# Gabrielcb/DaliID

Measured on AMD Instinct MI355X. Metric: images/sec (train step), higher is better.
Workload: dtype bf16; 1 GPU; configs[1]: ResNet-50 ReID bf16 256x128, PK batch 16x16=256 per GPU, center+proxy heads, Adam, EMA; global_batch=256, per_gpu_batch=256, parallelism=dp1

## Files before the change

daliid_amd/csrc/conv.hip:

```cpp
#include "gemm_tile.h"
#include "kernels.h"
#include <cstdlib>
#include <type_traits>
#include <vector>
#include <string>
#include <cstdio>

namespace dali {

__device__ __forceinline__ void decode_pixel(const GatherGeom& g, int p, int& n, int& ho, int& wo) {
    if (g.lhw >= 0 && g.lw >= 0) {
        n = p >> g.lhw;
        const int rem = p & ((1 << g.lhw) - 1);
        ho = rem >> g.lw;
        wo = rem & ((1 << g.lw) - 1);
    } else {
        const int hw = g.Hout * g.Wout;
        n = p / hw;
        const int rem = p - n * hw;
        ho = rem / g.Wout;
        wo = rem - ho * g.Wout;
    }
}

// ... 2294 lines not shown
    GRID_XCD,
    GRID_CLASSES,
    GRID_CUS,
    GRID_HALO,
    GRID_SPLITS,
    GRID_SPLITS8,
};
struct GemmKernel {
    const void* fn;
    int block;
    int lds;
    int tm, tn;
    GemmGrid grid;
    int plan_wgs = 0;
    int f1_rb = 0;
    mutable DeviceOnce once{};
};
template <class F> static const void* kfn(F* f) { return reinterpret_cast<const void*>(f); }
constexpr int ring_lds(int tm, int tn, int k_tile, int stages) { return (tm + tn) * k_tile * 2 * stages; }
constexpr int REG128_LDS = GemmCfg<128, 128, 1, 1, 1>::LDS_BYTES, REG64_LDS = GemmCfg<64, 256, 1, 1, 1>::LDS_BYTES;
constexpr int DMA128_LDS = REG128_LDS / 2 * 3, DMA64_LDS = REG64_LDS / 2 * 3;
constexpr int HALO64_LDS = (3 * 64 * 64 + HALO64_PX * 64) * 2;

static const GemmKernel
    CONV128_BN{kfn(&igemm_conv_kernel<128, 128, true>), 256, REG128_LDS, 128, 128, GRID_XCD},
    CONV128{kfn(&igemm_conv_kernel<128, 128, false>), 256, REG128_LDS, 128, 128, GRID_XCD},
    DMA128{kfn(&igemm_conv_dma_kernel<128, 128, 3>), 256, DMA128_LDS, 128, 128, GRID_XCD},
    DMA128_LIN{kfn(&igemm_conv_dma_kernel<128, 128, 3, 1>), 256, DMA128_LDS, 128, 128, GRID_XCD},
    DMA128_FUSED{kfn(&igemm_conv_dma_kernel<128, 128, 3, 3>), 256, DMA128_LDS, 128, 128, GRID_XCD},
    DMA128_CLS{kfn(&igemm_conv_dma_kernel<128, 128, 3, 4>), 256, DMA128_LDS, 128, 128, GRID_CLASSES},
// ... 11 lines not shown
    WG128_FUSED{kfn(&igemm_conv_wg_kernel<2, 4, 3, 3>), 512, ring_lds(128, 256, 32, 3), 128, 256, GRID_XCD},
    WG128_CLS{kfn(&igemm_conv_wg_kernel<2, 4, 3, 4>), 512, ring_lds(128, 256, 32, 3), 128, 256, GRID_CLASSES},
    WG256{kfn(&igemm_conv_wg_kernel<4, 4, 4>), 1024, ring_lds(256, 256, 32, 4), 256, 256, GRID_XCD},
    K64S{kfn(&igemm_conv_k64s_kernel<2, 4, 8, 3>), 1024, ring_lds(128, 256, 64, 3), 128, 256, GRID_XCD},
    K64S_LIN{kfn(&igemm_conv_k64s_kernel<2, 4, 8, 3, 4, 4, 1>), 1024, ring_lds(128, 256, 64, 3), 128, 256, GRID_XCD},
    K64S_LEAN{kfn(&igemm_conv_k64s_kernel<2, 4, 8, 3, 4, 4, 5>), 1024, ring_lds(128, 256, 64, 3), 128, 256, GRID_XCD},
    K64S_SRC2{kfn(&igemm_conv_k64s_kernel<2, 4, 8, 3, 4, 4, 0, true>), 1024, ring_lds(128, 256, 64, 3), 128, 256, GRID_XCD},
    K64{kfn(&igemm_conv_k64_kernel<4, 4, 2>), 1024, ring_lds(256, 256, 64, 2), 256, 256, GRID_XCD},
    K64_LIN{kfn(&igemm_conv_k64_kernel<4, 4, 2, 4, 4, 1>), 1024, ring_lds(256, 256, 64, 2), 256, 256, GRID_XCD},
    K64_FUSED{kfn(&igemm_conv_k64_kernel<4, 4, 2, 4, 4, 3>), 1024, ring_lds(256, 256, 64, 2), 256, 256, GRID_XCD},
    K64_CLS{kfn(&igemm_conv_k64_kernel<4, 4, 2, 4, 4, 4>), 1024, ring_lds(256, 256, 64, 2), 256, 256, GRID_CLASSES},
    K64_SRC2{kfn(&igemm_conv_k64_kernel<4, 4, 2, 4, 4, 0, true>), 1024, ring_lds(256, 256, 64, 2), 256, 256, GRID_XCD},
    K64_FUSED_SRC2{kfn(&igemm_conv_k64_kernel<4, 4, 2, 4, 4, 3, true>), 1024, ring_lds(256, 256, 64, 2), 256, 256, GRID_XCD},
    K64_320{kfn(&igemm_conv_k64_kernel<4, 4, 2, 4, 5, 1>), 1024, ring_lds(256, 320, 64, 2), 256, 320, GRID_XCD};

template <int RB, bool RES, bool OM, bool BITS, bool SRC2 = false>
static GemmKernel f1_kernel() {
    return {kfn(&fused1x1_persist_kernel<3, RB, RES, OM, BITS, SRC2>), (F1_NC + F1_NP + F1_NR) * 64, f1_lds_bytes(3, RB, RB == 2 ? 128 : F1_KMAX),
            F1_TM, F1_TN, GRID_CUS, 0, RB};
}
static const GemmKernel F1[2][2][2][2] = {
    {{{f1_kernel<2, false, false, false, true>(), f1_kernel<2, false, false, true>()}, {f1_kernel<2, false, true, false>(), f1_kernel<2, false, true, true>()}},
     {{f1_kernel<2, true, false, false>(), f1_kernel<2, true, false, true>()}, {f1_kernel<2, true, true, false>(), f1_kernel<2, true, true, true>()}}},
    {{{f1_kernel<1, false, false, false, true>(), f1_kernel<1, false, false, true>()}, {f1_kernel<1, false, true, false>(), f1_kernel<1, false, true, true>()}},
     {{f1_kernel<1, true, false, false>(), f1_kernel<1, true, false, true>()}, {f1_kernel<1, true, true, false>(), f1_kernel<1, true, true, true>()}}}};

static const GemmKernel
    WG_BN{kfn(&igemm_wgrad_kernel<true>), 256, 0, 128, 128, GRID_SPLITS},
    WG_PLAIN{kfn(&igemm_wgrad_kernel<false>), 256, 0, 128, 128, GRID_SPLITS},
    WG_3X3{kfn(&igemm_wgrad3x3_kernel<3>), 512, 3 * W3_STAGE * 2, 128, 9 * 64, GRID_SPLITS8, 256};
static const GemmKernel WG_DMA[2] = {
    {kfn(&igemm_wgrad_dma_kernel<false>), 256, 0, 128, 128, GRID_SPLITS8},
    {kfn(&igemm_wgrad_dma_kernel<true>), 256, 0, 128, 128, GRID_SPLITS8}};
static const GemmKernel WG_WG[2] = {
    {kfn(&igemm_wgrad_wg_kernel<2, 4, 3>), 512, ring_lds(128, 256, 32, 3), 128, 256, GRID_SPLITS8, 512},
    {kfn(&igemm_wgrad_wg_kernel<2, 4, 3, true>), 512, ring_lds(128, 256, 32, 3), 128, 256, GRID_SPLITS8, 512}};
static const GemmKernel WG_P[2][2] = {
    {{kfn(&igemm_wgrad_p_kernel<2, 4, 4, 4, 8, 6>), 1024, ring_lds(128, 256, 32, 6), 128, 256, GRID_SPLITS8, 256},
     {kfn(&igemm_wgrad_p_kernel<2, 4, 4, 4, 8, 6, true>), 1024, ring_lds(128, 256, 32, 6), 128, 256, GRID_SPLITS8, 256}},
    {{kfn(&igemm_wgrad_p_kernel<1, 4, 8, 4, 4, 6>), 512, ring_lds(128, 256, 32, 6), 128, 256, GRID_SPLITS8, 256},
// ... 2 lines not shown
struct GemmChoice {
    const GemmKernel* k = nullptr;
    int tiles_m = 0, tiles_n = 0, lds = 0, class_grid = 0;
    unsigned grid = 0;
    int rc = DALI_OK, why_arg = 0;
    const char* why = nullptr;
    GemmChoice() = default;
    GemmChoice(int rc_, const char* why_, int why_arg_ = 0) : rc(rc_), why_arg(why_arg_), why(why_) {}
    int refuse() const { set_error(why, why_arg); return rc; }
};
static GemmChoice gemm_place(const GemmKernel& k, int rows, int cols, int mult, int Ck) {
    GemmChoice c;
    c.k = &k;
    c.tiles_m = (rows + k.tm - 1) / k.tm;
    c.tiles_n = (cols + k.tn - 1) / k.tn;
    c.lds = k.f1_rb ? f1_lds_bytes(3, k.f1_rb, Ck) : k.lds;
    switch (k.grid) {
        case GRID_XCD: c.grid = xcd_tile_grid(c.tiles_m, c.tiles_n); break;
        case GRID_CLASSES: c.class_grid = xcd_tile_grid(c.tiles_m, c.tiles_n); c.grid = mult * c.class_grid; break;
        case GRID_CUS: c.grid = mult; break;
        case GRID_HALO: c.grid = c.tiles_n; break;
        case GRID_SPLITS: c.grid = c.tiles_m * c.tiles_n * mult; break;
        case GRID_SPLITS8: c.grid = (c.tiles_m * c.tiles_n * mult + 7) / 8 * 8; break;
    }
    return c;
}
template <class Args>
static int gemm_launch(hipStream_t st, const GemmChoice& c, Args& args) {
    const GemmKernel& k = *c.k;
    DeviceOnce::Guard once(k.once);
    if (k.lds > 64 * 1024 && once.first()) {
// ... 31 lines not shown
    if (!n_cus) {
        int dev = 0, v = 0;
        if (hipGetDevice(&dev) != hipSuccess || hipDeviceGetAttribute(&v, hipDeviceAttributeMultiprocessorCount, dev) != hipSuccess) { set_error("conv: device query failed"); return -1; }
        n_cus = v > 8 ? v & ~7 : 8;
    }
    return n_cus;
}
static bool f1_fills(int Cm, int P, int n_cus) {
    const int tiles_m = Cm / F1_TM, tiles_n = (P + F1_TN - 1) / F1_TN;
    return n_cus > 0 && (long long)tiles_m * tiles_n >= 2ll * n_cus && (n_cus / 8) % tiles_m == 0;
}
static bool cat_act_ok(int Cm, int c1, int c2, int P, int parts, int n_cus) {
    const int K = parts * (c1 + c2);
    if (parts != 1 && parts != 2) return false;
    if ((c1 & 63) || (c2 & 63) || (Cm % 128) || !dma_addressable((long long)P * Cm * 2) || !dma_addressable((long long)P * K * 2)) return false;
    if (K <= F1_KMAX) return f1_fills(Cm, P, n_cus);
    return parts == 1 && K >= 1024 && conv_pick_cfg(Cm, P, K) == CONV_256x256;
}
bool conv_cat_act_supported(int Cm, int c1, int c2, int P, int parts) { return cat_act_ok(Cm, c1, c2, P, parts, f1_cu_count()); }

static GemmChoice conv_choose(const IGemmArgs& a, int n_cus) {
    const GatherGeom& g = a.g;
    const bool in_bn = a.in_scale != nullptr, narrow = a.Cm <= 64, dma_ok = conv_dma_ok(a);
    const int K = g.nr * g.ns * g.Ck;
    const bool fused = a.out_scale || a.out_shift || a.out_relu || a.bits_out || a.out_mask || a.res_scale;
    const bool lin = a.act != 0 || a.O2 != nullptr || a.dact_pre != nullptr || a.row_scale != nullptr;
    int cfg = conv_pick_cfg(a.Cm, a.P, K);
    if (dma_ok && !a.stats && !fused && !g.sub && g.Ck % 64 == 0 && (a.Cm & 7) == 0 && conv_prefers_320(a.Cm, a.P, K)) cfg = CONV_256x320;
    if (!dma_ok && !in_bn && a.stats && (cfg == CONV_128x256 || cfg == CONV_256x256))
        return GemmChoice(DALI_ERR_LIMIT, "conv: tensors beyond 2 GiB are not supported together with the BatchNorm statistics epilogue");
    bool k64 = dma_ok && !narrow && g.Ck % 64 == 0;
    const bool narrow_k64 = dma_ok && narrow && g.Ck % 64 == 0 && K >= 512 && !a.X2;
    if (a.X2) {
        const bool fo_simple = !a.bits_out && !a.out_mask && !a.res_scale && !a.Res && (a.out_scale || a.out_shift || a.out_relu);
        const int xr = a.x_rep > 1 ? a.x_rep : 1, c2 = g.Ck / xr - a.Ck1;
        if (xr > 1 && !(fo_simple && g.Ck % xr == 0 && cat_act_ok(a.Cm, a.Ck1, c2, a.P, xr, n_cus) && g.Ck <= F1_KMAX))
            return GemmChoice(DALI_ERR_INVALID, "conv: split weight images (x_rep = %d) are served by the persistent streaming kernel only (K <= 256, >= 2 tiles per CU)", xr);
        if (fo_simple && ((a.Ck1 & 63) || (c2 & 63) || (a.Cm % 128)))
            return GemmChoice(DALI_ERR_INVALID, "conv: two operand tensors with a fused output stage need channel counts that are multiples of 64 and Cm %% 128 == 0");
        if (in_bn || !dma_ok || a.stats || (fused && !fo_simple) || lin || g.sub || g.R != 1 || g.S != 1 || g.stride != 1 || g.pad != 0 || a.Ck1 <= 0 ||
            a.Ck1 >= g.Ck / xr || (a.Ck1 & 31) || (c2 & 31) || (a.Cm & 7))
            return GemmChoice(DALI_ERR_INVALID, "conv: a second operand tensor needs a plain 1x1 / stride 1 problem with both channel counts multiples of 32");
        if ((a.Ck1 & 63) || (c2 & 63)) k64 = false;
    }
    if (k64 && cfg != CONV_256x320 && !((K >= 1024 && (cfg == CONV_256x256 || cfg == CONV_128x256)) || (K >= 768 && cfg == CONV_256x256))) k64 = false;
    if (a.X2 && !narrow && !(k64 && (cfg == CONV_256x256 || cfg == CONV_128x256))) { cfg = CONV_128; k64 = false; }
    auto use = [&](const GemmKernel& k) { return gemm_place(k, a.Cm, a.P, k.grid == GRID_CUS ? n_cus : (g.sub == 2 ? 4 : 1), g.Ck); };
    if (fused) {
        if (in_bn || !dma_ok || (a.Cm & 7) || lin)
            return GemmChoice(DALI_ERR_INVALID, "conv: the fused output stage needs Cm %% 8 == 0, tensors below 2 GiB, no operand transform and no linear-layer extras");
        if (plain_rows(g) && !g.sub && !a.res_mask && a.Cm % F1_TM == 0 && (g.Ck & 63) == 0 && g.Ck <= F1_KMAX && dma_addressable((long long)a.P * a.Cm * 2) &&
            (a.Res || a.out_mask || a.bits_out || a.X2)) {
            if (n_cus <= 0) return GemmChoice(DALI_ERR_HIP, "conv: device query failed");
            if (f1_fills(a.Cm, a.P, n_cus)) return use(F1[g.Ck > 128][a.Res != nullptr][a.out_mask != nullptr][a.bits_out != nullptr]);
        }
        const bool lean = !a.Res && !a.out_mask && !a.bits_out && !a.res_mask && !a.res_scale && !a.X2;
        if (lean && narrow_k64 && halo64_ok(a)) return use(HALO64_LEAN);
        if (lean && narrow) return use(DMA64_LEAN);
        if (lean && k64 && cfg == CONV_128x256 && !g.sub) return use(K64S_LEAN);
        if (a.X2) {
            if (!(k64 && cfg == CONV_256x256))
                return GemmChoice(DALI_ERR_INVALID, "conv: two operand tensors with a fused output stage need K <= 256 or a 256 x 256 k-tile-64 problem (K >= 1024, Cm >= 512, >= 16384 pixels)");
            return use(K64_FUSED_SRC2);
        }
        if (k64 && cfg == CONV_256x256) return use(K64_FUSED);
        return use(cfg == CONV_128x256 || cfg == CONV_256x256 ? WG128_FUSED : DMA128_FUSED);
    }
    if (g.sub && dma_ok && !narrow && !lin && (a.Cm & 7) == 0) {
        if (k64 && cfg == CONV_256x256) return use(K64_CLS);
// ... 313 lines not shown
}

extern "C" int dali_conv1x1_fused(dali_ctx* ctx, void* stream, const uint16_t* x, const uint16_t* w, uint16_t* y, int pixels, int cin, int cout,
                                  const float* out_scale, const float* out_shift, const float* bias, const uint16_t* residual, int out_relu,
                                  uint8_t* bits_out, const uint8_t* out_mask, const float* res_scale) {
    DALI_REQUIRE(ctx && x && w && y, "dali_conv1x1_fused: null argument");
    DALI_REQUIRE(cin % 32 == 0 && cout % 8 == 0 && pixels > 0, "dali_conv1x1_fused: cin %% 32, cout %% 8 (cin=%d cout=%d)", cin, cout);
    IGemmArgs a{};
    a.W = w; a.X = x; a.O = y; a.Res = residual; a.bias = bias;
    a.out_scale = out_scale; a.out_shift = out_shift; a.out_relu = out_relu; a.bits_out = bits_out; a.out_mask = out_mask; a.res_scale = res_scale;
    a.Cm = cout; a.P = pixels;
    fill_geom(a.g, 1, 1, pixels, cin, 1, pixels, 1, 1, 1, 0, 0);
    return launch_igemm_conv((hipStream_t)stream, a);
}

extern "C" int dali_conv1x1_cat(dali_ctx* ctx, void* stream, const uint16_t* x1, int c1, const uint16_t* x2, int c2, const uint16_t* w, const float* bias,
                                uint16_t* y, int pixels, int cout) {
    DALI_REQUIRE(ctx && x1 && x2 && w && y, "dali_conv1x1_cat: null argument");
    DALI_REQUIRE(c1 > 0 && c2 > 0 && c1 % 32 == 0 && c2 % 32 == 0 && cout % 8 == 0 && pixels > 0, "dali_conv1x1_cat: c1 %% 32, c2 %% 32, cout %% 8 (c1=%d c2=%d cout=%d)", c1, c2, cout);
    IGemmArgs a{};
    a.W = w; a.X = x1; a.X2 = x2; a.Ck1 = c1; a.O = y; a.bias = bias;
    a.Cm = cout; a.P = pixels;
    fill_geom(a.g, 1, 1, pixels, c1 + c2, 1, pixels, 1, 1, 1, 0, 0);
    return launch_igemm_conv((hipStream_t)stream, a);
}

extern "C" int dali_conv1x1_cat_act(dali_ctx* ctx, void* stream, const uint16_t* x1, int c1, const uint16_t* x2, int c2, const uint16_t* w, int weight_parts,
                                    const float* out_scale, const float* out_shift, int out_relu, uint16_t* y, int pixels, int cout) {
    DALI_REQUIRE(ctx && x1 && x2 && w && y && out_shift, "dali_conv1x1_cat_act: null argument");
    DALI_REQUIRE(c1 > 0 && c2 > 0 && c1 % 64 == 0 && c2 % 64 == 0 && cout % 128 == 0 && pixels > 0, "dali_conv1x1_cat_act: c1 %% 64, c2 %% 64, cout %% 128 (c1=%d c2=%d cout=%d)", c1, c2, cout);
// ... 80 lines not shown
```

daliid_amd/csrc/fused1x1.h:

```cpp
#pragma once

namespace dali {

__device__ __forceinline__ unsigned f1_pos_bits(uint32_t w) {
    const uint32_t p = ((w & 0x7fff7fffu) + 0x7fff7fffu) & ~w & 0x80008000u;
    return ((p >> 15) | (p >> 30)) & 3u;
}

template <int N> __device__ __forceinline__ void f1_vm_wait_imm() { asm volatile("s_waitcnt vmcnt(%0)" ::"n"(N) : "memory"); }
__device__ __forceinline__ void f1_vm_wait(int n) {
    switch (n) {
        case 1: f1_vm_wait_imm<1>(); break;
        case 2: f1_vm_wait_imm<2>(); break;
        case 3: f1_vm_wait_imm<3>(); break;
        case 4: f1_vm_wait_imm<4>(); break;
        case 5: f1_vm_wait_imm<5>(); break;
        case 6: f1_vm_wait_imm<6>(); break;
        case 7: f1_vm_wait_imm<7>(); break;
        case 8: f1_vm_wait_imm<8>(); break;
        case 9: f1_vm_wait_imm<9>(); break;
        case 10: f1_vm_wait_imm<10>(); break;
        case 11: f1_vm_wait_imm<11>(); break;
        case 12: f1_vm_wait_imm<12>(); break;
        case 13: f1_vm_wait_imm<13>(); break;
// ... 12 lines not shown
        case 26: f1_vm_wait_imm<26>(); break;
        case 27: f1_vm_wait_imm<27>(); break;
        case 28: f1_vm_wait_imm<28>(); break;
        default: f1_vm_wait_imm<0>(); break;
    }
}

__device__ __forceinline__ void f1_vm_wait_pieces(int n) {
    if (n == 17) f1_vm_wait_imm<17>();
    else if (n == 16) f1_vm_wait_imm<16>();
    else if (n == 1) f1_vm_wait_imm<1>();
    else f1_vm_wait_imm<0>();
}

constexpr int F1_TM = 128, F1_TN = 128, F1_NC = 8, F1_NP = 4, F1_NR = 2;
constexpr int F1_KMAX = 256;
constexpr int F1_R_BYTES = F1_TN * F1_TM * 2;
constexpr int F1_M_BYTES = F1_TN * F1_TM / 8;
constexpr int F1_C_BYTES = 3 * F1_TM * 4;
constexpr int f1_lds_bytes(int NS, int RB, int K) {
    return F1_TM * K * 2 + NS * F1_TN * 64 * 2 + RB * F1_R_BYTES + RB * F1_M_BYTES + F1_C_BYTES;
}

template <int F1_NS, int F1_RB, bool HAS_RES, bool HAS_OM, bool HAS_BITS, bool SRC2 = false>
__global__ __launch_bounds__((F1_NC + F1_NP + F1_NR) * 64) void fused1x1_persist_kernel(IGemmArgs a, int tiles_m, int tiles_n) {
    extern __shared__ __attribute__((aligned(16))) uint16_t smem[];
    const int K = a.g.Ck, KT = K >> 6, P = a.P, Cm = a.Cm;
    constexpr int STAGE = F1_TN * 64;
    uint16_t* const ring = smem + F1_TM * K;
    char* const rbuf = reinterpret_cast<char*>(ring + F1_NS * STAGE);
    char* const mbuf = rbuf + F1_RB * F1_R_BYTES;
    float* const cbuf = reinterpret_cast<float*>(mbuf + F1_RB * F1_M_BYTES);
    const int tid = threadIdx.x, lane = tid & 63;
    const int wave = __builtin_amdgcn_readfirstlane(tid >> 6);
    const int xcd = blockIdx.x & 7, slot = blockIdx.x >> 3, S = gridDim.x >> 3;
    const int n0 = (int)((long long)xcd * tiles_n / 8), n1 = (int)((long long)(xcd + 1) * tiles_n / 8);
    const int items = (n1 - n0) * tiles_m;
    const int T = slot < items ? (items - slot + S - 1) / S : 0;
    if (T == 0) return;
    const int GT = T * KT;
    auto tile_of = [&](int t, int& tm, int& tn) {
        const int q = slot + S * t, d = q / tiles_m;
        tn = n0 + d;
        tm = q - d * tiles_m;
    };

    if (wave >= F1_NC && wave < F1_NC + F1_NP) {
        const int pw = wave - F1_NC;
        const __amdgpu_buffer_rsrc_t rs_w = __builtin_amdgcn_make_buffer_rsrc(const_cast<uint16_t*>(a.W), 0, Cm * K * 2, 0x00020000);
        const int rep = SRC2 && a.x_rep > 1 ? a.x_rep : 1;
        const int Ck1 = SRC2 ? a.Ck1 : K, Ck2 = K / rep - Ck1;
        const __amdgpu_buffer_rsrc_t rs_x = __builtin_amdgcn_make_buffer_rsrc(const_cast<uint16_t*>(a.X), 0, (int)((long long)P * Ck1 * 2), 0x00020000);
        const __amdgpu_buffer_rsrc_t rs_x2 = __builtin_amdgcn_make_buffer_rsrc(const_cast<uint16_t*>(SRC2 ? a.X2 : a.X), 0, (int)((long long)P * (SRC2 ? Ck2 : Ck1) * 2), 0x00020000);
        const int r_in = lane >> 3;
        const int kc = (lane & 7) ^ (((pw & 1) << 2) | (r_in >> 1));
        constexpr int NPC = F1_TM / 8 / F1_NP;
        constexpr int PK = NPC;
        int issued = 0, it = 0, ik = 0, st_issue = 0;
        uint32_t a_off[NPC], b_off[NPC];
        auto set_tile = [&](int t) {
            int tm, tn;
            tile_of(t, tm, tn);
#pragma unroll
            for (int i = 0; i < NPC; ++i) {
                const int m = tm * F1_TM + 8 * (pw + F1_NP * i) + r_in;
                a_off[i] = (uint32_t)(m * K + kc * 8) * 2u;
                const int p = tn * F1_TN + 8 * (pw + F1_NP * i) + r_in;
                if constexpr (SRC2) b_off[i] = p < P ? (uint32_t)p : DMA_OOB;
                else b_off[i] = p < P ? (uint32_t)(p * K + kc * 8) * 2u : DMA_OOB;
            }
        };
        set_tile(0);
        for (int k = 0; k < KT; ++k)
#pragma unroll
            for (int i = 0; i < NPC; ++i)
                __builtin_amdgcn_raw_ptr_buffer_load_lds(rs_w, (lds_void_ptr)(smem + k * (F1_TM * 64) + (pw + F1_NP * i) * 512), 16, a_off[i] + (uint32_t)k * 128u, 0, 0, 0);
        auto issue_one = [&]() {
            uint16_t* sb = ring + st_issue * STAGE;
            st_issue = st_issue == F1_NS - 1 ? 0 : st_issue + 1;
            const uint32_t kb = (uint32_t)ik * 128u;
            if constexpr (SRC2) {
                const int kc0 = ik * 64;
                const bool second = kc0 >= rep * Ck1;
                const int pitch = second ? Ck2 : Ck1, cbase = (second ? (kc0 - rep * Ck1) % Ck2 : kc0 % Ck1) + kc * 8;
#pragma unroll
                for (int i = 0; i < NPC; ++i) {
                    const uint32_t off = b_off[i] == DMA_OOB ? DMA_OOB : (uint32_t)((int)b_off[i] * pitch + cbase) * 2u;
                    if (second) __builtin_amdgcn_raw_ptr_buffer_load_lds(rs_x2, (lds_void_ptr)(sb + (pw + F1_NP * i) * 512), 16, off, 0, 0, 0);
                    else __builtin_amdgcn_raw_ptr_buffer_load_lds(rs_x, (lds_void_ptr)(sb + (pw + F1_NP * i) * 512), 16, off, 0, 0, 0);
                }
            } else {
#pragma unroll
                for (int i = 0; i < NPC; ++i) {
                    const uint32_t off = b_off[i] == DMA_OOB ? DMA_OOB : b_off[i] + kb;
                    __builtin_amdgcn_raw_ptr_buffer_load_lds(rs_x, (lds_void_ptr)(sb + (pw + F1_NP * i) * 512), 16, off, 0, 0, 0);
                }
            }
            ++issued;
            if (++ik == KT) {
                ik = 0;
                if (++it < T) set_tile(it);
            }
        };
        auto fill = [&](int next_step) {
            const int lim = GT < next_step + F1_NS ? GT : next_step + F1_NS;
            while (issued < lim) issue_one();
        };
        fill(0);
        f1_vm_wait(PK * (issued - 1));
        __builtin_amdgcn_s_barrier();
// ... 10 lines not shown
                __builtin_amdgcn_s_barrier();
                if (stamp) { t_issue += s1 - s0; t_wait += s2 - s1; t_bar += __builtin_amdgcn_s_memrealtime() - s2; }
            }
            fill(g);
            __builtin_amdgcn_s_barrier();
            if (g < GT) f1_vm_wait(PK * (issued - 1 - g));
            __builtin_amdgcn_s_barrier();
        }
        if (stamp && lane == 0) {
            a.stamps[(size_t)blockIdx.x * 12 + 9] = t_issue; a.stamps[(size_t)blockIdx.x * 12 + 10] = t_wait; a.stamps[(size_t)blockIdx.x * 12 + 11] = t_bar;
        }
        return;
    }

    constexpr bool has_res = HAS_RES, has_om = HAS_OM, has_bits = HAS_BITS;
    if (wave >= F1_NC + F1_NP) {
        const int rw = wave - F1_NC - F1_NP;
        const __amdgpu_buffer_rsrc_t rs_r = __builtin_amdgcn_make_buffer_rsrc(const_cast<uint16_t*>(has_res ? a.Res : a.X), 0, has_res ? (int)((long long)P * Cm * 2) : 0, 0x00020000);
        const __amdgpu_buffer_rsrc_t rs_m = __builtin_amdgcn_make_buffer_rsrc(const_cast<uint8_t*>(has_om ? a.out_mask : reinterpret_cast<const uint8_t*>(a.X)), 0,
                                                                              has_om ? (int)((long long)P * Cm / 8) : 0, 0x00020000);
        constexpr int RP = F1_R_BYTES / 1024 / F1_NR;
        const int pieces = (has_res ? RP : 0) + (has_om ? 1 : 0);
        auto issue_rm = [&](int t) {
            int tm, tn;
            tile_of(t, tm, tn);
            char* rb = rbuf + (F1_RB == 2 ? (t & 1) : 0) * F1_R_BYTES;
            if (has_res) {
#pragma unroll
                for (int i = 0; i < RP; ++i) {
                    const int r = rw + F1_NR * i;
                    const int pix = 4 * r + (lane >> 4);
                    const int lc = (lane & 15) ^ (pix & 15);
// ... 16 lines not shown
                    if (k == 0 && t + 1 < T) issue_rm(t + 1);
                    if (k == KT - 1) { if (t + 1 < T) f1_vm_wait_pieces(pieces); else f1_vm_wait_imm<0>(); }
                } else {
                    if (k == 0 && t > 0) issue_rm(t);
                    if (k == KT - 1) f1_vm_wait_imm<0>();
                }
                __builtin_amdgcn_s_barrier();
            }
            __builtin_amdgcn_s_barrier();
            __builtin_amdgcn_s_barrier();
        }
        return;
    }

    const int wm = wave >> 2, wn = wave & 3;
    {
        int tm, tn;
        tile_of(0, tm, tn);
        if (tid < F1_TM) {
            const int c = tm * F1_TM + tid;
            cbuf[tid] = a.out_scale ? a.out_scale[c] : 1.f;
            cbuf[F1_TM + tid] = (a.out_shift ? a.out_shift[c] : 0.f) + (a.bias ? a.bias[c] : 0.f);
            cbuf[2 * F1_TM + tid] = a.res_scale ? a.res_scale[c] : 1.f;
        }
        asm volatile("s_waitcnt vmcnt(0) lgkmcnt(0)" ::: "memory");
    }
    const int frag_off = (lane & 15) * 64 + (((lane >> 4) ^ ((lane & 15) >> 1)) << 3);
    const int relu = a.out_relu;
    __builtin_amdgcn_s_barrier();
    int st_cur = 0;
    const bool stamp = a.stamps != nullptr && tid == 0;
    unsigned long long c_main = 0, c_mainbar = 0, c_e0 = 0, c_e0bar = 0, c_e1 = 0, c_e1bar = 0;
    const unsigned long long c_start = stamp ? __builtin_amdgcn_s_memrealtime() : 0;
    for (int t = 0; t < T; ++t) {
        int tm, tn;
        tile_of(t, tm, tn);
        f32x4_t acc[4][2];
#pragma unroll
        for (int i = 0; i < 4; ++i)
#pragma unroll
            for (int j = 0; j < 2; ++j) acc[i][j] = f32x4_t{0.f, 0.f, 0.f, 0.f};
        for (int k = 0; k < KT; ++k) {
            const unsigned long long s0 = stamp ? __builtin_amdgcn_s_memrealtime() : 0;
            const uint16_t* sb = ring + st_cur * STAGE;
            const uint16_t* sa = smem + k * (F1_TM * 64);
            st_cur = st_cur == F1_NS - 1 ? 0 : st_cur + 1;
#pragma unroll
            for (int h = 0; h < 2; ++h) {
                const int fo = frag_off ^ (h << 5);
                bf16x8_t fa[4];
#pragma unroll
                for (int i = 0; i < 4; ++i) fa[i] = *reinterpret_cast<const bf16x8_t*>(sa + (wm * 64 + i * 16) * 64 + fo);
#pragma unroll
                for (int j = 0; j < 2; ++j) {
                    const bf16x8_t fb = *reinterpret_cast<const bf16x8_t*>(sb + (wn * 32 + j * 16) * 64 + fo);
#pragma unroll
                    for (int i = 0; i < 4; ++i) acc[i][j] = __builtin_amdgcn_mfma_f32_16x16x32_bf16(fa[i], fb, acc[i][j], 0, 0, 0);
                }
            }
            asm volatile("s_waitcnt lgkmcnt(0)" ::: "memory");
            const unsigned long long s1 = stamp ? __builtin_amdgcn_s_memrealtime() : 0;
            __builtin_amdgcn_s_barrier();
            if (stamp) { c_main += s1 - s0; c_mainbar += __builtin_amdgcn_s_memrealtime() - s1; }
        }
        const unsigned long long e0s = stamp ? __builtin_amdgcn_s_memrealtime() : 0;
        char* rb = rbuf + (F1_RB == 2 ? (t & 1) : 0) * F1_R_BYTES;
        {
            auto slot_of = [&](int i, int j) -> uint2* {
                const int pix = wn * 32 + j * 16 + (lane & 15);
                const int chunk = wm * 8 + i * 2 + (lane >> 5);
                return reinterpret_cast<uint2*>(rb + pix * 256 + ((lane >> 4) & 1) * 8 + ((chunk ^ (pix & 15)) << 4));
            };
            const float lo = relu ? 0.f : -__builtin_huge_valf();
#pragma unroll
            for (int j = 0; j < 2; ++j) {
                uint2 rv[4];
                if (has_res) {
#pragma unroll
                    for (int i = 0; i < 4; ++i) rv[i] = *slot_of(i, j);
                }
#pragma unroll
                for (int i = 0; i < 4; ++i) {
// ... 13 lines not shown
        }
        asm volatile("s_waitcnt lgkmcnt(0)" ::: "memory");
        const unsigned long long e0e = stamp ? __builtin_amdgcn_s_memrealtime() : 0;
        __builtin_amdgcn_s_barrier();
        const unsigned long long e1s = stamp ? __builtin_amdgcn_s_memrealtime() : 0;
        const bool interior = (tn + 1) * F1_TN <= P;
        const char* mb = mbuf + (F1_RB == 2 ? (t & 1) : 0) * F1_M_BYTES;
        if (interior) {
            auto ld = [&](int itr) { const int s = itr * (F1_NC * 64) + tid, pix = s >> 4, chunk = s & 15;
                                     return *reinterpret_cast<const uint4*>(rb + pix * 256 + ((chunk ^ (pix & 15)) << 4)); };
            auto ldm = [&](int itr) -> unsigned { const int s = itr * (F1_NC * 64) + tid, pix = s >> 4, chunk = s & 15;
                                                   return has_om ? *reinterpret_cast<const uint8_t*>(mb + pix * 16 + chunk) : 0u; };
            auto put = [&](int itr, uint4 v, unsigned m) {
                const int s = itr * (F1_NC * 64) + tid, pix = s >> 4, chunk = s & 15;
                if (has_om) { v.x = gate_bf16x2(v.x, m); v.y = gate_bf16x2(v.y, m >> 2); v.z = gate_bf16x2(v.z, m >> 4); v.w = gate_bf16x2(v.w, m >> 6); }
                const size_t e = ((size_t)(tn * F1_TN + pix) * Cm + tm * F1_TM + chunk * 8);
                *reinterpret_cast<uint4*>(a.O + e) = v;
                if (has_bits) a.bits_out[e >> 3] = (uint8_t)(f1_pos_bits(v.x) | (f1_pos_bits(v.y) << 2) | (f1_pos_bits(v.z) << 4) | (f1_pos_bits(v.w) << 6));
            };
            if constexpr (has_res && has_om) {
                { const uint4 v0 = ld(0), v1 = ld(1); const unsigned k0 = ldm(0), k1 = ldm(1); put(0, v0, k0); put(1, v1, k1); }
                { const uint4 v2 = ld(2), v3 = ld(3); const unsigned k2 = ldm(2), k3 = ldm(3); put(2, v2, k2); put(3, v3, k3); }
            } else {
            const uint4 v0 = ld(0), v1 = ld(1), v2 = ld(2), v3 = ld(3);
            const unsigned k0 = ldm(0), k1 = ldm(1), k2 = ldm(2), k3 = ldm(3);
            put(0, v0, k0); put(1, v1, k1); put(2, v2, k2); put(3, v3, k3);
            }
        } else {
#pragma unroll
            for (int itr = 0; itr < 4; ++itr) {
                const int s = itr * (F1_NC * 64) + tid, pix = s >> 4, chunk = s & 15;
                uint4 v = *reinterpret_cast<const uint4*>(rb + pix * 256 + ((chunk ^ (pix & 15)) << 4));
                if (has_om) {
                    const unsigned m = *reinterpret_cast<const uint8_t*>(mb + pix * 16 + chunk);
                    v.x = gate_bf16x2(v.x, m); v.y = gate_bf16x2(v.y, m >> 2); v.z = gate_bf16x2(v.z, m >> 4); v.w = gate_bf16x2(v.w, m >> 6);
                }
                if (tn * F1_TN + pix < P) {
                    const size_t e = ((size_t)(tn * F1_TN + pix) * Cm + tm * F1_TM + chunk * 8);
                    *reinterpret_cast<uint4*>(a.O + e) = v;
                    if (has_bits) a.bits_out[e >> 3] = (uint8_t)(f1_pos_bits(v.x) | (f1_pos_bits(v.y) << 2) | (f1_pos_bits(v.z) << 4) | (f1_pos_bits(v.w) << 6));
                }
            }
        }
        asm volatile("s_waitcnt lgkmcnt(0)" ::: "memory");
        const unsigned long long e1e = stamp ? __builtin_amdgcn_s_memrealtime() : 0;
        __builtin_amdgcn_s_barrier();
        if (stamp) { c_e0 += e0e - e0s; c_e0bar += e1s - e0e; c_e1 += e1e - e1s; c_e1bar += __builtin_amdgcn_s_memrealtime() - e1e; }
    }
    if (stamp) {
        unsigned long long* o = a.stamps + (size_t)blockIdx.x * 12;
        o[0] = c_start; o[3] = __builtin_amdgcn_s_memrealtime(); o[1] = c_main; o[2] = c_mainbar; o[4] = c_e0; o[5] = c_e0bar; o[6] = c_e1; o[7] = c_e1bar; o[8] = (unsigned long long)T;
    }
}

}
```

include/daliid_debug.h:

```cpp
#ifndef DALIID_DEBUG_H
#define DALIID_DEBUG_H

#ifdef __cplusplus
extern "C" {
#endif

int dali_debug_reload_env(void);

int dali_debug_set_conv_stamps(void* dev_ptr);

int dali_debug_wgrad_splits(int Cm, int Ntot, int P, int taps, int halo_w);

int dali_debug_splitk_reduce(void* stream, const float* partial, float* out, long long elems, int splits, int accumulate);

struct dali_resnet;
int dali_debug_resnet_backward_block(struct dali_resnet* net, void* stream, const float* d_emb, int block);

#ifdef __cplusplus
}
#endif
#endif
```

Before: 17240 images/s.

## Hold 1x1 conv weights in registers to extend persistent fused kernel to K<=512

Adds a register-resident-weight variant of the persistent fused 1x1 conv kernel. Each compute wave loads its 16-row weight slice into VGPRs once, so LDS only holds the streamed activation ring. This lets the fused-epilogue streaming path serve K up to 512 instead of 256, with fewer producer waves and a new MFMA/epilogue layout. The cost is much higher register pressure (up to 16 uint4 per lane for K=512) and possible occupancy or spill problems. It also narrows output index math to 32-bit and adds a debug query for which kernel gets selected.

```diff
diff --git a/daliid_amd/csrc/conv.hip b/daliid_amd/csrc/conv.hip
--- a/daliid_amd/csrc/conv.hip
+++ b/daliid_amd/csrc/conv.hip
@@ -2332,6 +2332,7 @@
     GemmGrid grid;
     int plan_wgs = 0;
     int f1_rb = 0;
+    bool f1_regw = false;
     mutable DeviceOnce once{};
 };
 template <class F> static const void* kfn(F* f) { return reinterpret_cast<const void*>(f); }
@@ -2373,16 +2374,25 @@
     K64_FUSED_SRC2{kfn(&igemm_conv_k64_kernel<4, 4, 2, 4, 4, 3, true>), 1024, ring_lds(256, 256, 64, 2), 256, 256, GRID_XCD},
     K64_320{kfn(&igemm_conv_k64_kernel<4, 4, 2, 4, 5, 1>), 1024, ring_lds(256, 320, 64, 2), 256, 320, GRID_XCD};
 
-template <int RB, bool RES, bool OM, bool BITS, bool SRC2 = false>
+template <int RB, bool RES, bool OM, bool BITS, bool SRC2 = false, int KR = 0>
 static GemmKernel f1_kernel() {
-    return {kfn(&fused1x1_persist_kernel<3, RB, RES, OM, BITS, SRC2>), (F1_NC + F1_NP + F1_NR) * 64, f1_lds_bytes(3, RB, RB == 2 ? 128 : F1_KMAX),
-            F1_TM, F1_TN, GRID_CUS, 0, RB};
-}
-static const GemmKernel F1[2][2][2][2] = {
-    {{{f1_kernel<2, false, false, false, true>(), f1_kernel<2, false, false, true>()}, {f1_kernel<2, false, true, false>(), f1_kernel<2, false, true, true>()}},
-     {{f1_kernel<2, true, false, false>(), f1_kernel<2, true, false, true>()}, {f1_kernel<2, true, true, false>(), f1_kernel<2, true, true, true>()}}},
-    {{{f1_kernel<1, false, false, false, true>(), f1_kernel<1, false, false, true>()}, {f1_kernel<1, false, true, false>(), f1_kernel<1, false, true, true>()}},
-     {{f1_kernel<1, true, false, false>(), f1_kernel<1, true, false, true>()}, {f1_kernel<1, true, true, false>(), f1_kernel<1, true, true, true>()}}}};
+    return {kfn(&fused1x1_persist_kernel<3, RB, RES, OM, BITS, SRC2, KR>), f1_waves(KR) * 64, f1_lds_bytes(3, RB, KR ? 0 : RB == 2 ? F1_KMAX_LDSW : F1_KMAX_SRC2),
+            F1_TM, F1_TN, GRID_CUS, 0, RB, KR > 0};
+}
+static const GemmKernel F1_LDSW[2][2][2] = {
+    {{f1_kernel<2, false, false, false, true>(), f1_kernel<2, false, false, true>()}, {f1_kernel<2, false, true, false>(), f1_kernel<2, false, true, true>()}},
+    {{f1_kernel<2, true, false, false>(), f1_kernel<2, true, false, true>()}, {f1_kernel<2, true, true, false>(), f1_kernel<2, true, true, true>()}}};
+static const GemmKernel F1_SRC2_LONG = f1_kernel<1, false, false, false, true>();
+static const GemmKernel F1_REGW[2][7] = {
+    {f1_kernel<2, false, false, true, false, 4>(), f1_kernel<2, false, true, false, false, 4>(), f1_kernel<2, false, true, true, false, 4>(), f1_kernel<2, true, false, false, false, 4>(),
+     f1_kernel<2, true, false, true, false, 4>(), f1_kernel<2, true, true, false, false, 4>(), f1_kernel<2, true, true, true, false, 4>()},
+    {f1_kernel<2, false, false, true, false, 8>(), f1_kernel<2, false, true, false, false, 8>(), f1_kernel<2, false, true, true, false, 8>(), f1_kernel<2, true, false, false, false, 8>(),
+     f1_kernel<2, true, false, true, false, 8>(), f1_kernel<2, true, true, false, false, 8>(), f1_kernel<2, true, true, true, false, 8>()}};
+static const GemmKernel& f1_pick(int K, bool res, bool om, bool bits, bool src2) {
+    if (K <= F1_KMAX_LDSW) return F1_LDSW[res][om][bits];
+    if (src2) return F1_SRC2_LONG;
+    return F1_REGW[K > 256][4 * res + 2 * om + bits - 1];
+}
 
 static const GemmKernel
     WG_BN{kfn(&igemm_wgrad_kernel<true>), 256, 0, 128, 128, GRID_SPLITS},
@@ -2415,7 +2425,7 @@
     c.k = &k;
     c.tiles_m = (rows + k.tm - 1) / k.tm;
     c.tiles_n = (cols + k.tn - 1) / k.tn;
-    c.lds = k.f1_rb ? f1_lds_bytes(3, k.f1_rb, Ck) : k.lds;
+    c.lds = k.f1_rb ? f1_lds_bytes(3, k.f1_rb, k.f1_regw ? 0 : Ck) : k.lds;
     switch (k.grid) {
         case GRID_XCD: c.grid = xcd_tile_grid(c.tiles_m, c.tiles_n); break;
         case GRID_CLASSES: c.class_grid = xcd_tile_grid(c.tiles_m, c.tiles_n); c.grid = mult * c.class_grid; break;
@@ -2477,7 +2487,7 @@
     const int K = parts * (c1 + c2);
     if (parts != 1 && parts != 2) return false;
     if ((c1 & 63) || (c2 & 63) || (Cm % 128) || !dma_addressable((long long)P * Cm * 2) || !dma_addressable((long long)P * K * 2)) return false;
-    if (K <= F1_KMAX) return f1_fills(Cm, P, n_cus);
+    if (K <= F1_KMAX_SRC2) return f1_fills(Cm, P, n_cus);
     return parts == 1 && K >= 1024 && conv_pick_cfg(Cm, P, K) == CONV_256x256;
 }
 bool conv_cat_act_supported(int Cm, int c1, int c2, int P, int parts) { return cat_act_ok(Cm, c1, c2, P, parts, f1_cu_count()); }
@@ -2497,7 +2507,7 @@
     if (a.X2) {
         const bool fo_simple = !a.bits_out && !a.out_mask && !a.res_scale && !a.Res && (a.out_scale || a.out_shift || a.out_relu);
         const int xr = a.x_rep > 1 ? a.x_rep : 1, c2 = g.Ck / xr - a.Ck1;
-        if (xr > 1 && !(fo_simple && g.Ck % xr == 0 && cat_act_ok(a.Cm, a.Ck1, c2, a.P, xr, n_cus) && g.Ck <= F1_KMAX))
+        if (xr > 1 && !(fo_simple && g.Ck % xr == 0 && cat_act_ok(a.Cm, a.Ck1, c2, a.P, xr, n_cus) && g.Ck <= F1_KMAX_SRC2))
             return GemmChoice(DALI_ERR_INVALID, "conv: split weight images (x_rep = %d) are served by the persistent streaming kernel only (K <= 256, >= 2 tiles per CU)", xr);
         if (fo_simple && ((a.Ck1 & 63) || (c2 & 63) || (a.Cm % 128)))
             return GemmChoice(DALI_ERR_INVALID, "conv: two operand tensors with a fused output stage need channel counts that are multiples of 64 and Cm %% 128 == 0");
@@ -2512,10 +2522,10 @@
     if (fused) {
         if (in_bn || !dma_ok || (a.Cm & 7) || lin)
             return GemmChoice(DALI_ERR_INVALID, "conv: the fused output stage needs Cm %% 8 == 0, tensors below 2 GiB, no operand transform and no linear-layer extras");
-        if (plain_rows(g) && !g.sub && !a.res_mask && a.Cm % F1_TM == 0 && (g.Ck & 63) == 0 && g.Ck <= F1_KMAX && dma_addressable((long long)a.P * a.Cm * 2) &&
-            (a.Res || a.out_mask || a.bits_out || a.X2)) {
+        if (plain_rows(g) && !g.sub && !a.res_mask && a.Cm % F1_TM == 0 && (g.Ck & 63) == 0 && g.Ck <= (a.X2 ? F1_KMAX_SRC2 : F1_KMAX_REGW) &&
+            dma_addressable((long long)a.P * a.Cm * 2) && (a.Res || a.out_mask || a.bits_out || a.X2)) {
             if (n_cus <= 0) return GemmChoice(DALI_ERR_HIP, "conv: device query failed");
-            if (f1_fills(a.Cm, a.P, n_cus)) return use(F1[g.Ck > 128][a.Res != nullptr][a.out_mask != nullptr][a.bits_out != nullptr]);
+            if (f1_fills(a.Cm, a.P, n_cus)) return use(f1_pick(g.Ck, a.Res != nullptr, a.out_mask != nullptr, a.bits_out != nullptr, a.X2 != nullptr));
         }
         const bool lean = !a.Res && !a.out_mask && !a.bits_out && !a.res_mask && !a.res_scale && !a.X2;
         if (lean && narrow_k64 && halo64_ok(a)) return use(HALO64_LEAN);
@@ -2859,6 +2869,26 @@
     return launch_igemm_conv((hipStream_t)stream, a);
 }
 
+extern "C" int dali_debug_conv1x1_fused_kernel(int pixels, int cin, int cout, int has_residual, int has_out_mask, int has_bits, int flags) {
+    DALI_REQUIRE(cin > 0 && cin % 32 == 0 && cout > 0 && cout % 8 == 0 && pixels > 0, "dali_debug_conv1x1_fused_kernel: cin %% 32, cout %% 8 (cin=%d cout=%d)", cin, cout);
+    static const uint16_t tensor = 0; static const float coeff = 0.f; static uint8_t bytes = 0;
+    IGemmArgs a{};
+    a.W = &tensor; a.X = &tensor; a.O = const_cast<uint16_t*>(&tensor);
+    a.Res = has_residual ? &tensor : nullptr; a.out_mask = has_out_mask ? &bytes : nullptr; a.bits_out = has_bits ? &bytes : nullptr;
+    a.out_relu = flags & 1; a.out_scale = (flags & 2) ? &coeff : nullptr; a.out_shift = (flags & 4) ? &coeff : nullptr;
+    a.bias = (flags & 8) ? &coeff : nullptr; a.res_scale = (flags & 16) ? &coeff : nullptr;
+    a.Cm = cout; a.P = pixels;
+    fill_geom(a.g, 1, 1, pixels, cin, 1, pixels, 1, 1, 1, 0, 0);
+    GatherGeom& g = a.g;
+    g.sub = 0; g.oph = g.opw = 0; g.Hfull = g.Hout; g.Wfull = g.Wout;
+    g.r0 = 0; g.rstep = 1; g.nr = g.R; g.s0 = 0; g.sstep = 1; g.ns = g.S;
+    g.lw = ilog2_exact(g.Wout); g.lhw = ilog2_exact(g.Hout * g.Wout);
+    const GemmChoice c = conv_choose(a, f1_cu_count());
+    if (!c.k) return -1;
+    if (c.k->grid != GRID_CUS) return 0;
+    return c.k->f1_regw ? 2 : 1;
+}
+
 extern "C" int dali_conv1x1_cat(dali_ctx* ctx, void* stream, const uint16_t* x1, int c1, const uint16_t* x2, int c2, const uint16_t* w, const float* bias,
                                 uint16_t* y, int pixels, int cout) {
     DALI_REQUIRE(ctx && x1 && x2 && w && y, "dali_conv1x1_cat: null argument");
diff --git a/daliid_amd/csrc/fused1x1.h b/daliid_amd/csrc/fused1x1.h
--- a/daliid_amd/csrc/fused1x1.h
+++ b/daliid_amd/csrc/fused1x1.h
@@ -1,4 +1,5 @@
 #pragma once
+#include <type_traits>
 
 namespace dali {
 
@@ -50,7 +51,10 @@
 }
 
 constexpr int F1_TM = 128, F1_TN = 128, F1_NC = 8, F1_NP = 4, F1_NR = 2;
-constexpr int F1_KMAX = 256;
+constexpr int F1_NP_REGW = 2;
+constexpr int F1_KMAX_LDSW = 128;
+constexpr int F1_KMAX_REGW = 512;
+constexpr int F1_KMAX_SRC2 = 256;
 constexpr int F1_R_BYTES = F1_TN * F1_TM * 2;
 constexpr int F1_M_BYTES = F1_TN * F1_TM / 8;
 constexpr int F1_C_BYTES = 3 * F1_TM * 4;
@@ -58,12 +62,19 @@
     return F1_TM * K * 2 + NS * F1_TN * 64 * 2 + RB * F1_R_BYTES + RB * F1_M_BYTES + F1_C_BYTES;
 }
 
-template <int F1_NS, int F1_RB, bool HAS_RES, bool HAS_OM, bool HAS_BITS, bool SRC2 = false>
-__global__ __launch_bounds__((F1_NC + F1_NP + F1_NR) * 64) void fused1x1_persist_kernel(IGemmArgs a, int tiles_m, int tiles_n) {
+typedef uint32_t f1_u32x4_t __attribute__((ext_vector_type(4)));
+constexpr int f1_waves(int KR) { return F1_NC + (KR ? F1_NP_REGW : F1_NP) + F1_NR; }
+
+template <int F1_NS, int F1_RB, bool HAS_RES, bool HAS_OM, bool HAS_BITS, bool SRC2 = false, int KR = 0>
+__global__ __launch_bounds__(f1_waves(KR) * 64) void fused1x1_persist_kernel(IGemmArgs a, int tiles_m, int tiles_n) {
     extern __shared__ __attribute__((aligned(16))) uint16_t smem[];
+    constexpr bool REGW = KR > 0;
+    constexpr bool EXACT = KR == 8;
+    constexpr int NP = REGW ? F1_NP_REGW : F1_NP;
+    static_assert(!(REGW && SRC2) && (!REGW || F1_RB == 2), "register weights: one operand tensor, two result buffers");
     const int K = a.g.Ck, KT = K >> 6, P = a.P, Cm = a.Cm;
     constexpr int STAGE = F1_TN * 64;
-    uint16_t* const ring = smem + F1_TM * K;
+    uint16_t* const ring = smem + (REGW ? 0 : F1_TM * K);
     char* const rbuf = reinterpret_cast<char*>(ring + F1_NS * STAGE);
     char* const mbuf = rbuf + F1_RB * F1_R_BYTES;
     float* const cbuf = reinterpret_cast<float*>(mbuf + F1_RB * F1_M_BYTES);
@@ -81,7 +92,7 @@
         tm = q - d * tiles_m;
     };
 
-    if (wave >= F1_NC && wave < F1_NC + F1_NP) {
+    if (wave >= F1_NC && wave < F1_NC + NP) {
         const int pw = wave - F1_NC;
         const __amdgpu_buffer_rsrc_t rs_w = __builtin_amdgcn_make_buffer_rsrc(const_cast<uint16_t*>(a.W), 0, Cm * K * 2, 0x00020000);
         const int rep = SRC2 && a.x_rep > 1 ? a.x_rep : 1;
@@ -90,27 +101,32 @@
         const __amdgpu_buffer_rsrc_t rs_x2 = __builtin_amdgcn_make_buffer_rsrc(const_cast<uint16_t*>(SRC2 ? a.X2 : a.X), 0, (int)((long long)P * (SRC2 ? Ck2 : Ck1) * 2), 0x00020000);
         const int r_in = lane >> 3;
         const int kc = (lane & 7) ^ (((pw & 1) << 2) | (r_in >> 1));
-        constexpr int NPC = F1_TM / 8 / F1_NP;
+        constexpr int NPC = F1_TM / 8 / NP;
         constexpr int PK = NPC;
+        static_assert(PK * (F1_NS - 1) <= 28, "f1_vm_wait's table");
         int issued = 0, it = 0, ik = 0, st_issue = 0;
-        uint32_t a_off[NPC], b_off[NPC];
+        uint32_t b_off[NPC];
         auto set_tile = [&](int t) {
             int tm, tn;
             tile_of(t, tm, tn);
 #pragma unroll
             for (int i = 0; i < NPC; ++i) {
-                const int m = tm * F1_TM + 8 * (pw + F1_NP * i) + r_in;
-                a_off[i] = (uint32_t)(m * K + kc * 8) * 2u;
-                const int p = tn * F1_TN + 8 * (pw + F1_NP * i) + r_in;
+                const int p = tn * F1_TN + 8 * (pw + NP * i) + r_in;
                 if constexpr (SRC2) b_off[i] = p < P ? (uint32_t)p : DMA_OOB;
                 else b_off[i] = p < P ? (uint32_t)(p * K + kc * 8) * 2u : DMA_OOB;
             }
         };
         set_tile(0);
-        for (int k = 0; k < KT; ++k)
-#pragma unroll
-            for (int i = 0; i < NPC; ++i)
-                __builtin_amdgcn_raw_ptr_buffer_load_lds(rs_w, (lds_void_ptr)(smem + k * (F1_TM * 64) + (pw + F1_NP * i) * 512), 16, a_off[i] + (uint32_t)k * 128u, 0, 0, 0);
+        if constexpr (!REGW) {
+            int tm, tn;
+            tile_of(0, tm, tn);
+            for (int k = 0; k < KT; ++k)
+#pragma unroll
+                for (int i = 0; i < F1_TM / 8 / F1_NP; ++i) {
+                    const int m = tm * F1_TM + 8 * (pw + F1_NP * i) + r_in;
+                    __builtin_amdgcn_raw_ptr_buffer_load_lds(rs_w, (lds_void_ptr)(smem + k * (F1_TM * 64) + (pw + F1_NP * i) * 512), 16, (uint32_t)(m * K + kc * 8) * 2u + (uint32_t)k * 128u, 0, 0, 0);
+                }
+        }
         auto issue_one = [&]() {
             uint16_t* sb = ring + st_issue * STAGE;
             st_issue = st_issue == F1_NS - 1 ? 0 : st_issue + 1;
@@ -122,14 +138,14 @@
 #pragma unroll
                 for (int i = 0; i < NPC; ++i) {
                     const uint32_t off = b_off[i] == DMA_OOB ? DMA_OOB : (uint32_t)((int)b_off[i] * pitch + cbase) * 2u;
-                    if (second) __builtin_amdgcn_raw_ptr_buffer_load_lds(rs_x2, (lds_void_ptr)(sb + (pw + F1_NP * i) * 512), 16, off, 0, 0, 0);
-                    else __builtin_amdgcn_raw_ptr_buffer_load_lds(rs_x, (lds_void_ptr)(sb + (pw + F1_NP * i) * 512), 16, off, 0, 0, 0);
+                    if (second) __builtin_amdgcn_raw_ptr_buffer_load_lds(rs_x2, (lds_void_ptr)(sb + (pw + NP * i) * 512), 16, off, 0, 0, 0);
+                    else __builtin_amdgcn_raw_ptr_buffer_load_lds(rs_x, (lds_void_ptr)(sb + (pw + NP * i) * 512), 16, off, 0, 0, 0);
                 }
             } else {
 #pragma unroll
                 for (int i = 0; i < NPC; ++i) {
                     const uint32_t off = b_off[i] == DMA_OOB ? DMA_OOB : b_off[i] + kb;
-                    __builtin_amdgcn_raw_ptr_buffer_load_lds(rs_x, (lds_void_ptr)(sb + (pw + F1_NP * i) * 512), 16, off, 0, 0, 0);
+                    __builtin_amdgcn_raw_ptr_buffer_load_lds(rs_x, (lds_void_ptr)(sb + (pw + NP * i) * 512), 16, off, 0, 0, 0);
                 }
             }
             ++issued;
@@ -170,8 +186,8 @@
     }
 
     constexpr bool has_res = HAS_RES, has_om = HAS_OM, has_bits = HAS_BITS;
-    if (wave >= F1_NC + F1_NP) {
-        const int rw = wave - F1_NC - F1_NP;
+    if (wave >= F1_NC + NP) {
+        const int rw = wave - F1_NC - NP;
         const __amdgpu_buffer_rsrc_t rs_r = __builtin_amdgcn_make_buffer_rsrc(const_cast<uint16_t*>(has_res ? a.Res : a.X), 0, has_res ? (int)((long long)P * Cm * 2) : 0, 0x00020000);
         const __amdgpu_buffer_rsrc_t rs_m = __builtin_amdgcn_make_buffer_rsrc(const_cast<uint8_t*>(has_om ? a.out_mask : reinterpret_cast<const uint8_t*>(a.X)), 0,
                                                                               has_om ? (int)((long long)P * Cm / 8) : 0, 0x00020000);
@@ -218,6 +234,17 @@
     }
 
     const int wm = wave >> 2, wn = wave & 3;
+    f1_u32x4_t wreg[REGW ? 2 * KR : 1];
+    if constexpr (REGW) {
+        int tm, tn;
+        tile_of(0, tm, tn);
+        const uint16_t* wp = a.W + (size_t)(tm * F1_TM + wave * 16 + (lane & 15)) * K + (lane >> 4) * 8;
+#pragma unroll
+        for (int kb = 0; kb < 2 * KR; ++kb) {
+            wreg[kb] = f1_u32x4_t{0u, 0u, 0u, 0u};
+            if (kb * 32 < K) wreg[kb] = *reinterpret_cast<const f1_u32x4_t*>(wp + kb * 32);
+        }
+    }
     {
         int tm, tn;
         tile_of(0, tm, tn);
@@ -229,21 +256,53 @@
         }
         asm volatile("s_waitcnt vmcnt(0) lgkmcnt(0)" ::: "memory");
     }
+    if constexpr (REGW) {
+#pragma unroll
+        for (int kb = 0; kb < 2 * KR; ++kb) asm volatile("" : "+v"(wreg[kb]));
+    }
     const int frag_off = (lane & 15) * 64 + (((lane >> 4) ^ ((lane & 15) >> 1)) << 3);
     const int relu = a.out_relu;
     __builtin_amdgcn_s_barrier();
     int st_cur = 0;
-    const bool stamp = a.stamps != nullptr && tid == 0;
+    const bool stamp = a.stamps != nullptr && wave == 0;
     unsigned long long c_main = 0, c_mainbar = 0, c_e0 = 0, c_e0bar = 0, c_e1 = 0, c_e1bar = 0;
     const unsigned long long c_start = stamp ? __builtin_amdgcn_s_memrealtime() : 0;
     for (int t = 0; t < T; ++t) {
         int tm, tn;
         tile_of(t, tm, tn);
         f32x4_t acc[4][2];
+        f32x4_t racc[8];
 #pragma unroll
         for (int i = 0; i < 4; ++i)
 #pragma unroll
             for (int j = 0; j < 2; ++j) acc[i][j] = f32x4_t{0.f, 0.f, 0.f, 0.f};
+#pragma unroll
+        for (int j = 0; j < 8; ++j) racc[j] = f32x4_t{0.f, 0.f, 0.f, 0.f};
+        if constexpr (REGW) {
+#pragma unroll
+            for (int k = 0; k < KR; ++k) {
+                if (k < KT) {
+                    const unsigned long long s0 = stamp ? __builtin_amdgcn_s_memrealtime() : 0;
+                    const uint16_t* sb = ring + st_cur * STAGE;
+                    st_cur = st_cur == F1_NS - 1 ? 0 : st_cur + 1;
+#pragma unroll
+                    for (int h = 0; h < 2; ++h) {
+                        const int fo = frag_off ^ (h << 5);
+                        if constexpr (KR == 8) if (h == 1) __builtin_amdgcn_sched_barrier(0);
+                        bf16x8_t fb[8];
+#pragma unroll
+                        for (int j = 0; j < 8; ++j) fb[j] = *reinterpret_cast<const bf16x8_t*>(sb + (j * 16) * 64 + fo);
+#pragma unroll
+                        for (int j = 0; j < 8; ++j)
+                            racc[j] = __builtin_amdgcn_mfma_f32_16x16x32_bf16(__builtin_bit_cast(bf16x8_t, wreg[2 * k + h]), fb[j], racc[j], 0, 0, 0);
+                    }
+                    asm volatile("s_waitcnt lgkmcnt(0)" ::: "memory");
+                    const unsigned long long s1 = stamp ? __builtin_amdgcn_s_memrealtime() : 0;
+                    __builtin_amdgcn_s_barrier();
+                    if (stamp) { c_main += s1 - s0; c_mainbar += __builtin_amdgcn_s_memrealtime() - s1; }
+                }
+            }
+        } else
         for (int k = 0; k < KT; ++k) {
             const unsigned long long s0 = stamp ? __builtin_amdgcn_s_memrealtime() : 0;
             const uint16_t* sb = ring + st_cur * STAGE;
@@ -269,7 +328,53 @@
         }
         const unsigned long long e0s = stamp ? __builtin_amdgcn_s_memrealtime() : 0;
         char* rb = rbuf + (F1_RB == 2 ? (t & 1) : 0) * F1_R_BYTES;
-        {
+        if constexpr (REGW) {
+            auto slot_of = [&](int j) -> uint2* {
+                const int pix = j * 16 + (lane & 15);
+                const int chunk = wave * 2 + (lane >> 5);
+                return reinterpret_cast<uint2*>(rb + pix * 256 + ((lane >> 4) & 1) * 8 + ((chunk ^ (pix & 15)) << 4));
+            };
+            const int c = wave * 16 + (lane >> 4) * 4;
+            const float4 s4 = *reinterpret_cast<const float4*>(cbuf + c), h4 = *reinterpret_cast<const float4*>(cbuf + F1_TM + c);
+            float4 r4 = make_float4(1.f, 1.f, 1.f, 1.f);
+            if (has_res) r4 = *reinterpret_cast<const float4*>(cbuf + 2 * F1_TM + c);
+            const float lo = relu ? 0.f : -__builtin_huge_valf();
+            auto beat1 = [&](auto relu_c) {
+            constexpr int G = KR == 8 ? 2 : 4;
+#pragma unroll
+            for (int g4 = 0; g4 < 8 / G; ++g4) {
+                uint2 rv[G];
+                if (has_res) {
+#pragma unroll
+                    for (int jj = 0; jj < G; ++jj) rv[jj] = *slot_of(g4 * G + jj);
+                }
+#pragma unroll
+                for (int jj = 0; jj < G; ++jj) {
+                    const int j = g4 * G + jj;
+                    float v0, v1, v2, v3;
+                    if constexpr (EXACT) {
+                        v0 = racc[j][0] * s4.x + h4.x; v1 = racc[j][1] * s4.y + h4.y; v2 = racc[j][2] * s4.z + h4.z; v3 = racc[j][3] * s4.w + h4.w;
+                        if (has_res) {
+                            v0 += r4.x * bf16_bits_to_f32(rv[jj].x & 0xffffu); v1 += r4.y * bf16_bits_to_f32(rv[jj].x >> 16);
+                            v2 += r4.z * bf16_bits_to_f32(rv[jj].y & 0xffffu); v3 += r4.w * bf16_bits_to_f32(rv[jj].y >> 16);
+                        }
+                        if constexpr (decltype(relu_c)::value) { v0 = fmaxf(v0, 0.f); v1 = fmaxf(v1, 0.f); v2 = fmaxf(v2, 0.f); v3 = fmaxf(v3, 0.f); }
+                    } else {
+                        v0 = __builtin_fmaf(racc[j][0], s4.x, h4.x); v1 = __builtin_fmaf(racc[j][1], s4.y, h4.y);
+                        v2 = __builtin_fmaf(racc[j][2], s4.z, h4.z); v3 = __builtin_fmaf(racc[j][3], s4.w, h4.w);
+                        if (has_res) {
+                            v0 = __builtin_fmaf(r4.x, bf16_bits_to_f32(rv[jj].x & 0xffffu), v0); v1 = __builtin_fmaf(r4.y, bf16_bits_to_f32(rv[jj].x >> 16), v1);
+                            v2 = __builtin_fmaf(r4.z, bf16_bits_to_f32(rv[jj].y & 0xffffu), v2); v3 = __builtin_fmaf(r4.w, bf16_bits_to_f32(rv[jj].y >> 16), v3);
+                        }
+                        v0 = fmaxf(v0, lo); v1 = fmaxf(v1, lo); v2 = fmaxf(v2, lo); v3 = fmaxf(v3, lo);
+                    }
+                    *slot_of(j) = make_uint2(pack_bf16x2(v0, v1), pack_bf16x2(v2, v3));
+                }
+            }
+            };
+            if (EXACT && relu) beat1(std::true_type{});
+            else beat1(std::false_type{});
+        } else {
             auto slot_of = [&](int i, int j) -> uint2* {
                 const int pix = wn * 32 + j * 16 + (lane & 15);
                 const int chunk = wm * 8 + i * 2 + (lane >> 5);
@@ -313,7 +418,7 @@
             auto put = [&](int itr, uint4 v, unsigned m) {
                 const int s = itr * (F1_NC * 64) + tid, pix = s >> 4, chunk = s & 15;
                 if (has_om) { v.x = gate_bf16x2(v.x, m); v.y = gate_bf16x2(v.y, m >> 2); v.z = gate_bf16x2(v.z, m >> 4); v.w = gate_bf16x2(v.w, m >> 6); }
-                const size_t e = ((size_t)(tn * F1_TN + pix) * Cm + tm * F1_TM + chunk * 8);
+                const uint32_t e = (uint32_t)((tn * F1_TN + pix) * Cm + tm * F1_TM + chunk * 8);
                 *reinterpret_cast<uint4*>(a.O + e) = v;
                 if (has_bits) a.bits_out[e >> 3] = (uint8_t)(f1_pos_bits(v.x) | (f1_pos_bits(v.y) << 2) | (f1_pos_bits(v.z) << 4) | (f1_pos_bits(v.w) << 6));
             };
@@ -335,7 +440,7 @@
                     v.x = gate_bf16x2(v.x, m); v.y = gate_bf16x2(v.y, m >> 2); v.z = gate_bf16x2(v.z, m >> 4); v.w = gate_bf16x2(v.w, m >> 6);
                 }
                 if (tn * F1_TN + pix < P) {
-                    const size_t e = ((size_t)(tn * F1_TN + pix) * Cm + tm * F1_TM + chunk * 8);
+                    const uint32_t e = (uint32_t)((tn * F1_TN + pix) * Cm + tm * F1_TM + chunk * 8);
                     *reinterpret_cast<uint4*>(a.O + e) = v;
                     if (has_bits) a.bits_out[e >> 3] = (uint8_t)(f1_pos_bits(v.x) | (f1_pos_bits(v.y) << 2) | (f1_pos_bits(v.z) << 4) | (f1_pos_bits(v.w) << 6));
                 }
@@ -346,7 +451,7 @@
         __builtin_amdgcn_s_barrier();
         if (stamp) { c_e0 += e0e - e0s; c_e0bar += e1s - e0e; c_e1 += e1e - e1s; c_e1bar += __builtin_amdgcn_s_memrealtime() - e1e; }
     }
-    if (stamp) {
+    if (stamp && lane == 0) {
         unsigned long long* o = a.stamps + (size_t)blockIdx.x * 12;
         o[0] = c_start; o[3] = __builtin_amdgcn_s_memrealtime(); o[1] = c_main; o[2] = c_mainbar; o[4] = c_e0; o[5] = c_e0bar; o[6] = c_e1; o[7] = c_e1bar; o[8] = (unsigned long long)T;
     }
diff --git a/include/daliid_debug.h b/include/daliid_debug.h
--- a/include/daliid_debug.h
+++ b/include/daliid_debug.h
@@ -11,6 +11,8 @@
 
 int dali_debug_wgrad_splits(int Cm, int Ntot, int P, int taps, int halo_w);
 
+int dali_debug_conv1x1_fused_kernel(int pixels, int cin, int cout, int has_residual, int has_out_mask, int has_bits, int flags);
+
 int dali_debug_splitk_reduce(void* stream, const float* partial, float* out, long long elems, int splits, int accumulate);
 
 struct dali_resnet;
```

Measured after the change: 17310 images/s (median of 6 runs). Within noise of the previous version (+0.4%).
